# StefanSko/mcmc-db

Hardware: AMD Instinct MI355X
Metric: validated param-draws/sec (higher is better)
Workload: dtype f64; 1 GPU; single posteriordb-shaped model, 4x10000x100 synthetic draws per GPU (BASELINE config 1; AR(1) chains, ties and a shifted chain; SURVEY 8(d) C1); layout=pcn, statistics=mean,std,q5,q50,q95,split_rhat,ess_bulk,ess_tail

## Files before the change

include/mcmcref_hip.h:

```cpp
#ifndef MCMCREF_HIP_H
#define MCMCREF_HIP_H

#include <stddef.h>
#include <stdint.h>

#ifdef __cplusplus
extern "C" {
#endif

#define MCR_VERSION 100

#define MCR_OK 0
#define MCR_EINVAL (-1)
#define MCR_EMINCHAINS (-2)
#define MCR_EMINCHAINS_ARG (-3)
#define MCR_ENONFINITE (-4)
#define MCR_EHIP (-5)
#define MCR_ENOMEM (-6)
#define MCR_ENODEVICE (-7)
#define MCR_ECOMM (-8)
#define MCR_ELAYOUT (-9)
#define MCR_EFALLBACK (-10)

#define MCR_F64 0
// ... 8 lines not shown
    double* std;
    double* q;
    double* median;
    double* rhat;
    double* rhat_bulk;
    double* rhat_tail;
    double* ess_bulk;
    double* ess_tail;
    int64_t* lag_bulk;
    int64_t* lag_tail;
    int64_t* q_lo;
} mcr_summary;

typedef struct mcr_kernel_time {
    char name[48];
    int64_t launches;
    double total_ms;
} mcr_kernel_time;

int mcr_version(void);
int mcr_device_count(void);
int mcr_init(int device, mcr_ctx** out);
void mcr_free(mcr_ctx* ctx);
const char* mcr_last_error(const mcr_ctx* ctx);
int mcr_set_workspace_limit(mcr_ctx* ctx, size_t bytes);

int mcr_plan_chunks(mcr_ctx* ctx, int64_t C, int64_t N, int64_t P, int64_t stride_c, int64_t stride_n, int64_t stride_p,
                    int diagnostics, int64_t* params_per_chunk);

int mcr_plan_chunks_chains(mcr_ctx* ctx, const int64_t* chain_off, int C, int64_t P, int diagnostics,
                           int64_t* params_per_chunk);

int mcr_rho_guard_count(mcr_ctx* ctx, int64_t* rederived);

int mcr_dev_alloc(mcr_ctx* ctx, size_t bytes, void** dptr);
int mcr_dev_free(mcr_ctx* ctx, void* dptr);
int mcr_memcpy_h2d(mcr_ctx* ctx, void* dptr, const void* hptr, size_t bytes);
int mcr_memcpy_d2h(mcr_ctx* ctx, void* hptr, const void* dptr, size_t bytes);
int mcr_sync(mcr_ctx* ctx);

int mcr_summarize(mcr_ctx* ctx, const void* draws, int dtype, int64_t C, int64_t N, int64_t P,
                  int64_t stride_c, int64_t stride_n, int64_t stride_p, int min_chains,
                  const double* quantiles, int n_q, mcr_summary* out);
int mcr_summarize_dev(mcr_ctx* ctx, const void* draws_dev, int dtype, int64_t C, int64_t N,
                      int64_t P, int64_t stride_c, int64_t stride_n, int64_t stride_p,
                      int min_chains, const double* quantiles, int n_q, mcr_summary* out);
#define MCR_MAX_INFLIGHT 8
int mcr_summarize_enqueue(mcr_ctx* ctx, const void* draws_dev, int dtype, int64_t C, int64_t N,
                          int64_t P, int64_t stride_c, int64_t stride_n, int64_t stride_p,
                          int min_chains, const double* quantiles, int n_q, mcr_summary* out);
int mcr_summarize_wait(mcr_ctx* ctx);
int mcr_summarize_wait_one(mcr_ctx* ctx);

typedef struct mcr_model_desc {
    const void* draws_dev;
    int dtype;
    int min_chains;
    int64_t C, N, P;
    int64_t stride_c, stride_n, stride_p;
} mcr_model_desc;
int mcr_summarize_models(mcr_ctx* ctx, const mcr_model_desc* models, int n_models, const double* quantiles,
                         int n_q, mcr_summary* outs);

int mcr_diagnose_chains(mcr_ctx* ctx, const double* pooled, const int64_t* chain_off, int C,
                        int min_chains, mcr_summary* out, double* z_bulk, double* z_tail,
                        double* rank_bulk, double* rank_tail);
// ... 247 lines not shown
```

mcmc-db_amd/csrc/mcr_api.hip:

```cpp
#include "../../include/mcmcref_hip.h"

#include <hip/hip_runtime.h>

#include <algorithm>
#include <cmath>
#include <cstdarg>
#include <cstdio>
#include <cstdlib>
#include <cstring>
#include <fcntl.h>
#include <sys/stat.h>
#include <unistd.h>
#include <atomic>
#include <chrono>
#include <exception>
#include <memory>
#include <thread>
#include <unordered_map>
#include <string>
#include <functional>
#include <new>
#include <vector>

#include "mcr_kernels.hpp"
// ... 549 lines not shown
    if (lds_spl > 60 * 1024)
        HIP_TRY(ctx, hipFuncSetAttribute(reinterpret_cast<const void*>(&k_splitters<KT, MVT>),
                                         hipFuncAttributeMaxDynamicSharedMemorySize, (int)lds_spl));
    LAUNCH(ctx, K_SPLITTERS, (k_splitters<KT, MVT>), dim3((unsigned)a.pc), dim3(1024), lds_spl, keys, (const double*)a.samp,
           a.M, a.bk_k, a.bk_B, a.bk_D, a.bk_R, a.cut, a.boff);
    return MCR_OK;
}
template <typename KT>
int launch_splitters(mcr_ctx* ctx, const PipeIn& a, const KT* keys)
{
    const int S = a.bk_k * (int)(a.bk_R / 64);
    if (S <= 1024 || ctx->splitters_pairwise) return launch_splitters_v<KT, 0>(ctx, a, keys);
    if (S <= 2048) return launch_splitters_v<KT, 2>(ctx, a, keys);
    if (S <= 4096) return launch_splitters_v<KT, 4>(ctx, a, keys);
    return launch_splitters_v<KT, 8>(ctx, a, keys);
}

struct Sorted {
    double* keys; void* pos;
    double* keys_free; void* pos_free;
    bool ranked;
};

template <typename IdxT>
int sort_stage_t(mcr_ctx* ctx, PipeIn& a, Sorted& out)
{
    const i64 M = a.M, pc = a.pc;
    const unsigned py = (unsigned)pc;
    constexpr size_t lds_tile = sort_lds_bytes<IdxT>(kTile);
    const bool bucket = a.bk_B > 0;
    double* const samp1 = (bucket && a.bk_R == kTile) ? a.samp : (double*)nullptr;
    if (a.x_f32) {
        LAUNCH(ctx, K_TILE_SORT, (k_tile_sort<kTileNT, kTileVT, IdxT, float>), dim3((unsigned)a.ntiles, py), dim3(kTileNT),
               lds_tile, (const float*)a.X, M, a.kA, (IdxT*)a.iA, a.part, (int)a.ntiles, samp1);
    } else {
        LAUNCH(ctx, K_TILE_SORT, (k_tile_sort<kTileNT, kTileVT, IdxT, double>), dim3((unsigned)a.ntiles, py), dim3(kTileNT),
               lds_tile, (const double*)a.X, M, a.kA, (IdxT*)a.iA, a.part, (int)a.ntiles, samp1);
    }
    double *kin = a.kA, *kout = a.kB;
    IdxT *iin = (IdxT*)a.iA, *iout = (IdxT*)a.iB;
    const unsigned nblk = (unsigned)((M + kTile - 1) / kTile);
    const i64 Rstop = bucket ? a.bk_R : M;
    for (i64 R = kTile; R < Rstop; R *= 2) {
        LAUNCH(ctx, K_MERGE, (k_merge<kMergeNT, kMergeVT, false, IdxT>), dim3(nblk, py), dim3(kMergeNT), lds_tile + 256,
               (const double*)kin, (const IdxT*)iin, kout, iout, M, R, (double*)nullptr, pc,
               QArgs{}, (u32*)nullptr, (const i64*)nullptr);
        std::swap(kin, kout);
        std::swap(iin, iout);
    }
    if (bucket) {
        if (a.bk_R != kTile)
            LAUNCH(ctx, K_SPLITTERS, k_sample_runs<double>, dim3((unsigned)a.bk_k, py), dim3(256), 0, (const double*)kin, M,
                   a.bk_R, a.samp);
        {
            const int rc = launch_splitters<double>(ctx, a, (const double*)kin);
            if (rc) return rc;
        }
        const unsigned pgrp = (unsigned)((pc + 7) / 8 * 8);
        LAUNCH(ctx, K_BUCKET_MERGE, (k_bucket_merge<kMergeNT, kMergeVT, IdxT>), dim3(pgrp * (unsigned)a.bk_B), dim3(kMergeNT),
               lds_tile, (const double*)kin, (const IdxT*)iin, kout, iout, M, a.bk_k, a.bk_B, (const u32*)a.cut,
               (const u32*)a.boff, a.do_diag ? a.zb : (u32*)nullptr, pc, a.bk_R);
        std::swap(kin, kout);
        std::swap(iin, iout);
    }
    out = Sorted{kin, iin, kout, iout, bucket};
    return MCR_OK;
}

int sort_stage_rec(mcr_ctx* ctx, PipeIn& a, Sorted& out)
{
// ... 499 lines not shown
        const int v = atoi(env);
        ctx->n_lanes = v < 1 ? 1 : (v > MCR_MAX_INFLIGHT ? MCR_MAX_INFLIGHT : v);
    }
    if (const char* env = getenv("MCR_IO_PIECE_KB")) {
        const long v = atol(env);
        ctx->io_piece = (size_t)(v < 64 ? 64 : (v > (1 << 20) ? (1 << 20) : v)) << 10;
    }
    if (const char* env = getenv("MCR_IO_THREADS")) {
        const int v = atoi(env);
        ctx->io_threads = v < 1 ? 1 : (v > 64 ? 64 : v);
    }
    e = hipSetDevice(device);
    for (int l = 0; l < ctx->n_lanes && e == hipSuccess; ++l)
        e = hipStreamCreateWithFlags(&ctx->lanes[l].stream, hipStreamNonBlocking);
    for (int l = 0; l < ctx->n_lanes && e == hipSuccess; ++l) {
        e = hipStreamCreateWithFlags(&ctx->lanes[l].aux, hipStreamNonBlocking);
        if (e == hipSuccess) e = hipEventCreateWithFlags(&ctx->lanes[l].fork, hipEventDisableTiming);
        if (e == hipSuccess) e = hipEventCreateWithFlags(&ctx->lanes[l].join, hipEventDisableTiming);
    }
    if (e == hipSuccess) e = hipStreamCreateWithFlags(&ctx->copy_stream, hipStreamNonBlocking);
    if (e != hipSuccess) {
        mcr_free(ctx);
        return fail(nullptr, MCR_EHIP, "device %d init failed: %s", device, hipGetErrorString(e));
    }
    use_lane(ctx, 0);
    size_t mb = 8192;
    if (const char* env = getenv("MCR_WORKSPACE_MB")) { const long v = atol(env); if (v > 0) mb = (size_t)v; }
    ctx->ws_limit = mb << 20;
    if (const char* env = getenv("MCR_F32_RECORDS")) ctx->f32_records = atoi(env) != 0;
    if (const char* env = getenv("MCR_FFT")) ctx->fft_on = atoi(env) != 0;
    if (const char* env = getenv("MCR_SPLITTERS_PAIRWISE")) ctx->splitters_pairwise = atoi(env) != 0;
    if (const char* env = getenv("MCR_FORK")) ctx->fork_lone = atoi(env) != 0;
    if (const char* env = getenv("MCR_RHO_BAND")) { const double v = atof(env); if (v >= 0.0 && v < 1.0) ctx->rho_band = v; }
    if (ctx->guard_count.reserve(ctx, sizeof(unsigned)) != MCR_OK ||
        hipMemsetAsync(ctx->guard_count.p, 0, sizeof(unsigned), ctx->stream) != hipSuccess ||
        hipStreamSynchronize(ctx->stream) != hipSuccess) {
        mcr_free(ctx);
        return fail(nullptr, MCR_ENOMEM, "device %d: cannot allocate the guard counter", device);
    }
    *out = ctx;
    return MCR_OK;
}

void mcr_free(mcr_ctx* ctx)
{
    if (!ctx) return;
    hipSetDevice(ctx->device);
    sync_all(ctx);
    prof_resolve(ctx);
    for (hipEvent_t e : ctx->free_ev) hipEventDestroy(e);
    for (Slot& s : ctx->slots) if (s.done) hipEventDestroy(s.done);
    if (ctx->copy_stream) hipStreamDestroy(ctx->copy_stream);
    delete ctx;
}

int mcr_rho_guard_count(mcr_ctx* ctx, int64_t* rederived)
{
    if (!ctx || !rederived) return fail(ctx, MCR_EINVAL, "NULL argument");
    hipSetDevice(ctx->device);
    sync_all(ctx);
    unsigned v = 0;
    HIP_TRY(ctx, hipMemcpy(&v, ctx->guard_count.p, sizeof(unsigned), hipMemcpyDeviceToHost));
    *rederived = (int64_t)v;
    return MCR_OK;
}

int mcr_set_workspace_limit(mcr_ctx* ctx, size_t bytes)
{
    if (!ctx) return fail(nullptr, MCR_EINVAL, "ctx is NULL");
    if (bytes < (1u << 20)) return fail(ctx, MCR_EINVAL, "workspace limit must be at least 1 MiB");
    ctx->ws_limit = bytes;
    return MCR_OK;
}

int mcr_plan_chunks(mcr_ctx* ctx, int64_t C, int64_t N, int64_t P, int64_t sc, int64_t sn, int64_t sp, int diagnostics,
                    int64_t* params_per_chunk)
{
    if (!ctx || !params_per_chunk) return fail(ctx, MCR_EINVAL, "mcr_plan_chunks: NULL argument");
    if (C <= 0 || N <= 0 || P <= 0) { *params_per_chunk = 0; return MCR_OK; }
    ChunkPlan cp;
    const int rc = plan_chunks(ctx, shape_regular(C, N), P, needs_ingest(C, N, P, sc, sn, sp), diagnostics != 0, cp);
    if (rc) return rc;
    *params_per_chunk = cp.pcmax;
    return MCR_OK;
}

int mcr_dev_alloc(mcr_ctx* ctx, size_t bytes, void** dptr)
{
    if (!ctx || !dptr) return fail(ctx, MCR_EINVAL, "NULL argument");
    HIP_TRY(ctx, hipSetDevice(ctx->device));
    HIP_TRY(ctx, hipMalloc(dptr, bytes ? bytes : 1));
    return MCR_OK;
}
int mcr_dev_free(mcr_ctx* ctx, void* dptr)
{
    if (!ctx) return fail(nullptr, MCR_EINVAL, "ctx is NULL");
// ... 2980 lines not shown
```

mcmc-db_amd/csrc/mcr_kernels.hpp:

```cpp
#pragma once
#include <type_traits>
#include "mcr_device.hpp"
#include "mcr_sortnet.h"

namespace mcr {

enum ResField {
    R_MEAN = 0, R_STD, R_MEDIAN, R_RHAT, R_RHAT_BULK, R_RHAT_TAIL, R_ESS_BULK, R_ESS_TAIL,
    R_LAG_BULK, R_LAG_TAIL, R_BAD, R_Q0
};

#ifndef MCR_WCOMB
#define MCR_WCOMB 1
#endif
constexpr bool kWriteCombine = MCR_WCOMB != 0;

struct QArgs {
    int nq;
    i64 lo[32];
    double g[32];
    const void* xt = nullptr;
    int xf32 = 0;
};

// ... 264 lines not shown
    constexpr unsigned long long kLowQuads = 0x0F0F0F0F0F0F0F0Full;
    lane_pair_stage<0x141, true, kLowQuads>(k, ix);
    lane_pair_stage<0x4E, false, kLowPairs>(k, ix);
    lane_pair_stage<0xB1, false, kEvenLanes>(k, ix);
    lane_bitonic_merge16(k, ix);
#endif
}

template <int VT>
__device__ __forceinline__ void serial_merge(const double* skey, int a0, int na, int b0, int nb, int ai,
                                             int bi, int nout, double (&k)[VT], int (&src)[VT])
{
    int pa = a0 + ai, pb = b0 + bi;
    const int ea = a0 + na, eb = b0 + nb;
    double ak = skey[pos16(pa)], bk = skey[pos16(pb)];
#pragma unroll
    for (int i = 0; i < VT; ++i) {
        if (i < nout) {
            const bool takeA = (pb >= eb) | ((pa < ea) & !(bk < ak));
            k[i] = takeA ? ak : bk;
            src[i] = takeA ? pa : pb;
            pa += takeA ? 1 : 0;
            pb += takeA ? 0 : 1;
            const int pn = takeA ? pa : pb;
            const double nv = skey[pos16(pn)];
            ak = takeA ? nv : ak;
            bk = takeA ? bk : nv;
        } else {
            src[i] = 0;
        }
    }
}

template <typename IdxT> constexpr size_t sort_lds_bytes(int T) { return (size_t)T * (8 + sizeof(IdxT)); }

template <int NT, int VT, typename IdxT, typename XT>
__global__ __launch_bounds__(NT) void k_tile_sort(const XT* __restrict__ X, i64 M,
                                                  double* __restrict__ keys, IdxT* __restrict__ idx,
                                                  double* __restrict__ part, int ntiles,
                                                  double* __restrict__ samp)
{
    constexpr int T = NT * VT;
    extern __shared__ __attribute__((aligned(16))) char smem[];
    double* skey = reinterpret_cast<double*>(smem);
    IdxT* sidx = reinterpret_cast<IdxT*>(skey + T);
    double* red = skey;

    const int tid = threadIdx.x, tile = blockIdx.x;
    const i64 p = blockIdx.y;
    const i64 base = (i64)tile * T;
    const int count = (int)((M - base < (i64)T) ? M - base : (i64)T);
    const XT* src = X + p * M + base;

    const bool full = count == T;
    double k[VT];
    u32 ix[VT];
    double bad = 0.0;
    auto load = [&](auto full_c) {
        constexpr bool FULL = decltype(full_c)::value;
#pragma unroll
        for (int i = 0; i < VT; ++i) {
            const int e = i * NT + tid;
            const bool live = FULL || e < count;
            const double v = (double)src[FULL ? e : min(e, count - 1)];
            k[i] = live ? v : INFINITY;
            ix[i] = live ? (u32)(base + e) : 0xFFFFFFFFu;
            bad += (live && !isfinite(v)) ? 1.0 : 0.0;
        }
    };
    if (full) load(std::true_type{}); else load(std::false_type{});
    thread_sort<VT>(k, ix);
    constexpr bool kLaneLevels = MCR_TILE_DPP_LEVELS >= 2 && VT == 16;
    if constexpr (kLaneLevels) lane_merge_levels_16_to_64(k, ix);
// ... 25 lines not shown
            sidx[posi(e)] = (IdxT)ix[i];
        }
        __syncthreads();
    }

    auto write_out = [&](auto full_c) {
        constexpr bool FULL = decltype(full_c)::value;
#pragma nounroll
        for (int e = tid; e < (FULL ? T : count); e += NT) {
            keys[p * M + base + e] = skey[pos16(e)];
            idx[p * M + base + e] = sidx[posi(e)];
        }
    };
    if (full) write_out(std::true_type{}); else write_out(std::false_type{});
    if (samp != nullptr && tid < T / 64) {
        const int e = 64 * tid + 63;
        samp[(p * ntiles + tile) * (T / 64) + tid] = (e < count) ? skey[pos16(e)] : INFINITY;
    }
    __syncthreads();
    double s1 = 0.0, s2 = 0.0, e1 = 0.0, mt = 0.0;
    auto moments = [&](auto full_c) {
        constexpr bool FULL = decltype(full_c)::value;
        const int nlive = count - tid * VT;
#pragma unroll
        for (int i = 0; i < VT; ++i) s1 += (FULL || i < nlive) ? k[i] : 0.0;
        s1 = block_sum<NT>(s1, red);
        mt = s1 / (double)count;
#pragma unroll
        for (int i = 0; i < VT; ++i) { const double d = (FULL || i < nlive) ? k[i] - mt : 0.0; s2 = fma(d, d, s2); e1 += d; }
    };
    if (full) moments(std::true_type{}); else moments(std::false_type{});
    block_sum3<NT>(s2, e1, bad, red);
    if (tid == 0) store_slice_moments(part + (p * ntiles + tile) * kMomRec, mt, e1, s2, bad, (double)count);
}

template <int NT, int VT>
__device__ __forceinline__ void scatter_codes_by_line(u32* __restrict__ zrow, i64 M, int total, const u32 (&hcode)[VT],
                                                      const u32 (&hpos)[VT], u32* cnt_code, unsigned short* spos, u32* swt)
{
    constexpr int kMaxLines = 2048, PER = kMaxLines / NT > 0 ? kMaxLines / NT : 1;
    static_assert(NT * PER >= kMaxLines, "every line counter has an owner in the scan");
    const int tid = threadIdx.x;
    const int nlines = (int)((M + 31) >> 5);
    u32* scnt = cnt_code;
    u32* scode = cnt_code + 2112;
    __syncthreads();
    for (int i = tid; i <= nlines; i += NT) scnt[i] = 0u;
    __syncthreads();
    u32 rk[VT];
#pragma unroll
    for (int i = 0; i < VT; ++i) rk[i] = (tid * VT + i < total) ? atomicAdd(&scnt[hpos[i] >> 5], 1u) : 0u;
    __syncthreads();
    {
        u32 c[PER], tsum = 0;
#pragma unroll
        for (int j = 0; j < PER; ++j) { const int q = tid * PER + j; c[j] = (q < nlines) ? scnt[q] : 0u; tsum += c[j]; }
        u32 wtot;
        const u32 wex = wave_excl_scan_u32(tsum, wtot);
        if ((tid & 63) == 0) swt[tid >> 6] = wtot;
        __syncthreads();
        u32 base = wex;
        for (int w = 0; w < (tid >> 6); ++w) base += swt[w];
#pragma unroll
        for (int j = 0; j < PER; ++j) { const int q = tid * PER + j; if (q < nlines) scnt[q] = base; base += c[j]; }
    }
    __syncthreads();
// ... 777 lines not shown
```

mcmc-db_amd/csrc/mcr_sort32.hpp:

```cpp
#pragma once
#include "mcr_kernels.hpp"

namespace mcr {

__device__ __forceinline__ u32 rec_key(u64 r) { return (u32)(r >> 32); }
__device__ __forceinline__ u32 rec_pos(u64 r) { return (u32)r; }

template <int VT>
__device__ __forceinline__ void thread_sort_rec(u64 (&r)[VT])
{
    static_assert(VT == 16 || VT == 8, "sorting networks exist for 16 and 8 items per lane");
#define MCR_CE(a, b)                                         \
    {                                                        \
        const bool sw = r[b] < r[a];                         \
        const u64 lo = sw ? r[b] : r[a], hi = sw ? r[a] : r[b]; \
        r[a] = lo; r[b] = hi;                                \
    }
    if constexpr (VT == 16) { MCR_NET16(MCR_CE) } else { MCR_NET8(MCR_CE) }
#undef MCR_CE
}

template <int CTRL>
__device__ __forceinline__ u64 dpp_u64(u64 v)
{
    return ((u64)dpp_u32<CTRL>((u32)(v >> 32)) << 32) | (u64)dpp_u32<CTRL>((u32)v);
}
__device__ __forceinline__ u64 select_by_mask(u64 a, u64 b, unsigned long long m)
{
    return ((u64)select_by_mask((u32)(a >> 32), (u32)(b >> 32), m) << 32) | (u64)select_by_mask((u32)a, (u32)b, m);
}

template <int CTRL, bool MIRROR, unsigned long long MIN_LANES>
__device__ __forceinline__ void lane_pair_stage_rec(u64 (&r)[16])
{
    auto exchange = [](u64& own, u64 o) {
        const unsigned long long lt = __builtin_amdgcn_ballot_w64(o < own), gt = __builtin_amdgcn_ballot_w64(own < o);
        own = select_by_mask(own, o, (lt & MIN_LANES) | (gt & ~MIN_LANES));
    };
#pragma unroll
    for (int i = 0; i < (MIRROR ? 8 : 16); ++i) {
        const int s = MIRROR ? 15 - i : i;
        const u64 o_i = dpp_u64<CTRL>(r[s]);
        if (MIRROR) {
            const u64 o_s = dpp_u64<CTRL>(r[i]);
            exchange(r[s], o_s);
        }
        exchange(r[i], o_i);
    }
}

__device__ __forceinline__ void lane_bitonic_merge16_rec(u64 (&r)[16])
{
#define MCR_CE(a, b)                                         \
    {                                                        \
        const bool sw = r[b] < r[a];                         \
        const u64 lo = sw ? r[b] : r[a], hi = sw ? r[a] : r[b]; \
        r[a] = lo; r[b] = hi;                                \
    }
    MCR_BITONIC16(MCR_CE)
#undef MCR_CE
}

__device__ __forceinline__ void lane_merge_levels_rec(u64 (&r)[16])
{
    constexpr unsigned long long kEvenLanes = 0x5555555555555555ull, kLowPairs = 0x3333333333333333ull,
                                 kLowQuads = 0x0F0F0F0F0F0F0F0Full;
    lane_pair_stage_rec<0xB1, true, kEvenLanes>(r);
    lane_bitonic_merge16_rec(r);
    lane_pair_stage_rec<0x1B, true, kLowPairs>(r);
    lane_pair_stage_rec<0xB1, false, kEvenLanes>(r);
    lane_bitonic_merge16_rec(r);
    lane_pair_stage_rec<0x141, true, kLowQuads>(r);
    lane_pair_stage_rec<0x4E, false, kLowPairs>(r);
    lane_pair_stage_rec<0xB1, false, kEvenLanes>(r);
    lane_bitonic_merge16_rec(r);
}

template <int VT, int LIM = 0>
__device__ __forceinline__ void serial_merge_rec(const u64* srec, int a0, int na, int b0, int nb, int ai, int bi,
                                                 int nout, u64 (&out)[VT])
{
    int pa = a0 + ai, pb = b0 + bi;
    const int ea = a0 + na, eb = b0 + nb;
    auto slot = [](int e) { return pos16(LIM > 0 ? min(e, LIM) : e); };
    u64 ar = srec[slot(pa)], br = srec[slot(pb)];
#pragma unroll
    for (int i = 0; i < VT; ++i) {
        if (i < nout) {
            const bool takeA = (pb >= eb) | ((pa < ea) & !(br < ar));
            out[i] = takeA ? ar : br;
            pa += takeA ? 1 : 0;
            pb += takeA ? 0 : 1;
            const int pn = takeA ? pa : pb;
            const u64 nv = srec[slot(pn)];
            ar = takeA ? nv : ar;
            br = takeA ? br : nv;
        } else {
            out[i] = kRecPad;
        }
    }
}

constexpr size_t rec_lds_bytes(int T) { return (size_t)(T + 2) * 8; }

template <int NT, int VT>
__global__ __launch_bounds__(NT) void k_tile_sort32(const float* __restrict__ X, i64 M, u64* __restrict__ recs,
                                                    double* __restrict__ part, int ntiles, double* __restrict__ samp)
{
    constexpr int T = NT * VT;
    extern __shared__ __attribute__((aligned(16))) char smem[];
    u64* srec = reinterpret_cast<u64*>(smem);
    double* red = reinterpret_cast<double*>(smem);

    const int tid = threadIdx.x, tile = blockIdx.x;
    const i64 p = blockIdx.y;
    const i64 base = (i64)tile * T;
    const int count = (int)((M - base < (i64)T) ? M - base : (i64)T);
    const float* src = X + p * M + base;

    const bool full = count == T;
    u64 r[VT];
    double bad = 0.0;
    auto load = [&](auto full_c) {
        constexpr bool FULL = decltype(full_c)::value;
#pragma unroll
        for (int i = 0; i < VT; ++i) {
            const int e = i * NT + tid;
            const bool live = FULL || e < count;
            const float v = src[FULL ? e : min(e, count - 1)];
            bad += (live && !isfinite(v)) ? 1.0 : 0.0;
            r[i] = live ? (((u64)f32_key(v) << 32) | (u64)(u32)(base + e)) : kRecPad;
        }
    };
    if (full) load(std::true_type{}); else load(std::false_type{});
// ... 251 lines not shown
```

mcmc-db_amd/mcmc_ref_hip/_ffi.py:

```python
from __future__ import annotations

import collections
import contextlib
import ctypes as C
import math
import os
import threading
import time
from pathlib import Path

import numpy as np

MCR_OK = 0
MCR_EINVAL, MCR_EMINCHAINS, MCR_EMINCHAINS_ARG, MCR_ENONFINITE = -1, -2, -3, -4
MCR_EHIP, MCR_ENOMEM, MCR_ENODEVICE, MCR_ECOMM, MCR_ELAYOUT = -5, -6, -7, -8, -9
MCR_EFALLBACK = -10
MCR_F64, MCR_F32 = 0, 1
MCR_MAX_QUANTILES = 32
MCR_MAX_INFLIGHT = 8

_PKG = Path(__file__).resolve().parent
DEFAULT_LIB = _PKG.parent / "lib" / "libmcmcref_hip.so"


# ... 48 lines not shown


class PqColumn(C.Structure):
    _fields_ = [("name", C.c_char_p), ("type", C.c_int), ("src_kind", C.c_int), ("src_dev", C.c_void_p),
                ("stride", C.c_int64), ("seq_div", C.c_int64), ("seq_mod", C.c_int64)]


def pq_column(name: str, type_: int, src, stride: int = 1, kind: int | None = None) -> tuple:
    return (name, type_, kind, src, stride, 1, 1)


def pq_sequence(name: str, type_: int, div: int = 1, mod: int = INT64_MAX) -> tuple:
    return (name, type_, MCR_PQW_SEQ, None, 0, div, mod)


class IdColumns(C.Structure):
    _fields_ = [("chain_dev", C.c_void_p), ("draw_dev", C.c_void_p), ("rows", C.c_int64)]


class KernelTime(C.Structure):
    _fields_ = [("name", C.c_char * 48), ("launches", C.c_int64), ("total_ms", C.c_double)]


_I64 = C.c_int64
_TENSOR = [C.c_void_p, C.c_int, _I64, _I64, _I64, _I64, _I64, _I64]
SYMBOLS = {
    "mcr_version": (C.c_int, []),
    "mcr_device_count": (C.c_int, []),
    "mcr_init": (C.c_int, [C.c_int, C.POINTER(C.c_void_p)]),
    "mcr_free": (None, [C.c_void_p]),
    "mcr_last_error": (C.c_char_p, [C.c_void_p]),
    "mcr_set_workspace_limit": (C.c_int, [C.c_void_p, C.c_size_t]),
    "mcr_rho_guard_count": (C.c_int, [C.c_void_p, C.POINTER(C.c_int64)]),
    "mcr_plan_chunks": (C.c_int, [C.c_void_p] + [C.c_int64] * 6 + [C.c_int, C.POINTER(C.c_int64)]),
    "mcr_plan_chunks_chains": (C.c_int, [C.c_void_p, _ip, C.c_int, _I64, C.c_int, C.POINTER(C.c_int64)]),
    "mcr_dev_alloc": (C.c_int, [C.c_void_p, C.c_size_t, C.POINTER(C.c_void_p)]),
    "mcr_dev_free": (C.c_int, [C.c_void_p, C.c_void_p]),
    "mcr_memcpy_h2d": (C.c_int, [C.c_void_p, C.c_void_p, C.c_void_p, C.c_size_t]),
    "mcr_memcpy_d2h": (C.c_int, [C.c_void_p, C.c_void_p, C.c_void_p, C.c_size_t]),
    "mcr_sync": (C.c_int, [C.c_void_p]),
    "mcr_summarize": (C.c_int, [C.c_void_p] + _TENSOR + [C.c_int, _dp, C.c_int, C.POINTER(Summary)]),
    "mcr_summarize_dev": (C.c_int, [C.c_void_p] + _TENSOR + [C.c_int, _dp, C.c_int, C.POINTER(Summary)]),
    "mcr_summarize_enqueue": (C.c_int, [C.c_void_p] + _TENSOR + [C.c_int, _dp, C.c_int, C.POINTER(Summary)]),
    "mcr_summarize_models": (C.c_int, [C.c_void_p, C.POINTER(ModelDesc), C.c_int, _dp, C.c_int, C.POINTER(Summary)]),
    "mcr_summarize_wait": (C.c_int, [C.c_void_p]),
    "mcr_summarize_wait_one": (C.c_int, [C.c_void_p]),
    "mcr_diagnose_chains": (C.c_int, [C.c_void_p, _dp, _ip, C.c_int, C.c_int, C.POINTER(Summary),
                                      _dp, _dp, _dp, _dp]),
    "mcr_summarize_chains_enqueue": (C.c_int, [C.c_void_p, C.c_void_p, _I64, _ip, C.c_int, _I64, C.c_int, _dp, C.c_int,
                                               C.POINTER(Summary)]),
    "mcr_summarize_chains_dev": (C.c_int, [C.c_void_p, C.c_void_p, _I64, _ip, C.c_int, _I64, C.c_int, _dp, C.c_int,
                                           C.POINTER(Summary)]),
    "mcr_basic_stats": (C.c_int, [C.c_void_p, C.c_void_p, C.c_int, _I64, _dp, _dp]),
    "mcr_moments_dev": (C.c_int, [C.c_void_p] + _TENSOR + [_dp, _dp]),
    "mcr_compare": (C.c_int, [C.c_void_p, _dp, _dp, _I64, C.c_double, _dp, C.POINTER(C.c_uint8)]),
    "mcr_two_sample": (C.c_int, [C.c_void_p, _dp, _I64, _dp, _I64, _I64, _dp, _dp]),
    "mcr_sliced_two_sample": (C.c_int, [C.c_void_p, _dp, _I64, _dp, _I64, _I64, _dp, _dp, _I64, _dp, _dp, _dp, _dp]),
    "mcr_sliced_two_sample_dev": (C.c_int, [C.c_void_p, C.c_void_p, _I64, C.c_void_p, _I64, _I64, _dp, _dp, _I64, _dp, _dp,
                                            _dp, _dp]),
    "mcr_sliced_plan": (C.c_int, [C.c_void_p, _I64, _I64, _I64, _I64, C.POINTER(C.c_int64)]),
    "mcr_nested_rhat": (C.c_int, [C.c_void_p] + _TENSOR + [C.POINTER(C.c_int32), C.POINTER(Nested)]),
    "mcr_nested_rhat_dev": (C.c_int, [C.c_void_p] + _TENSOR + [C.POINTER(C.c_int32), C.POINTER(Nested)]),
    "mcr_nested_plan": (C.c_int, [C.c_void_p, C.c_int] + [_I64] * 7 + [C.POINTER(C.c_int64)]),
    "mcr_covariance": (C.c_int, [C.c_void_p, _dp, _I64, _I64, _dp]),
    "mcr_covariance_dev": (C.c_int, [C.c_void_p, C.c_void_p, _I64, _I64, C.c_void_p]),
    "mcr_profile_enable": (C.c_int, [C.c_void_p, C.c_int]),
# ... 929 lines not shown
        arrs = {n: np.full(max(P, 1), np.nan) for n in NESTED_FIELDS}
        out = Nested(**{n: _as_dp(a) for n, a in arrs.items()})
        self._check(fn(self.handle, ptr, *targs, ids.ctypes.data_as(C.POINTER(C.c_int32)), C.byref(out)))
        return {n: a[:P] for n, a in arrs.items()}

    def nested_params_per_chunk(self, t: "DeviceTensor", K: int) -> int:
        v = C.c_int64(0)
        self._check(self.lib.mcr_nested_plan(self.handle, *t.targs, int(K), C.byref(v)))
        return int(v.value)

    def covariance(self, draws) -> np.ndarray:
        x = np.ascontiguousarray(draws, dtype=np.float64)
        if x.ndim != 2:
            raise ValueError("draws must be 2-D [P][M]")
        P = x.shape[0]
        cov = np.full((max(P, 1), max(P, 1)), np.nan)
        self._check(self.lib.mcr_covariance(self.handle, _as_dp(x), x.shape[1], P, _as_dp(cov)))
        return cov[:P, :P] if P else np.empty((0, 0))

    def params_per_chunk(self, t: "DeviceTensor", diagnostics: bool = True) -> int:
        _, C_, N, P, sc, sn, sp = t.targs
        v = C.c_int64(0)
        if t.chain_off is not None:
            self._check(self.lib.mcr_plan_chunks_chains(self.handle, _as_ip(t.chain_off), C_, P, int(diagnostics), C.byref(v)))
            return int(v.value)
        self._check(self.lib.mcr_plan_chunks(self.handle, C_, N, P, sc, sn, sp, int(diagnostics), C.byref(v)))
        return int(v.value)

    def rho_guard_count(self) -> int:
        v = C.c_int64(0)
        self._check(self.lib.mcr_rho_guard_count(self.handle, C.byref(v)))
        return int(v.value)

    def profile(self, on: bool):
        self._check(self.lib.mcr_profile_enable(self.handle, 1 if on else 0))

    def profile_reset(self):
        self._check(self.lib.mcr_profile_reset(self.handle))

    def profile_get(self) -> dict:
        arr = (KernelTime * 64)()
        n = C.c_int(0)
        self._check(self.lib.mcr_profile_get(self.handle, arr, 64, C.byref(n)))
        return {arr[i].name.decode(): {"launches": int(arr[i].launches), "total_ms": float(arr[i].total_ms)}
                for i in range(min(n.value, 64))}


def pipeline(ctx: Context, jobs, owns: bool = False):
    if ctx.inflight:
        ctx.wait()
    window = collections.deque()
    try:
        for tag, t, kw in jobs:
            try:
                window.append((tag, t, ctx.enqueue(t, **kw)))
            except McrError as exc:
                window.append((tag, t, exc))
            if len(window) == MCR_MAX_INFLIGHT:
                yield _retire(ctx, window, owns)
        while window:
            yield _retire(ctx, window, owns)
    finally:
        if window:
            try:
                ctx.wait()
            except McrError:
# ... 66 lines not shown
```

Before: 26.37 billion param-draws/s.

## Sort tile keys as packed 64-bit records with slot index, fallback on violations

The tile sort now packs each key and its 12-bit tile slot into a single double-sized record. The sorting network, DPP lane merges and LDS merge passes therefore move one 8-byte value instead of a key plus a separate index. The dropped low mantissa bits are restored afterwards from a side LDS array. If the rebuilt keys are not in order, the tile is re-sorted with the original key/index path and a device counter is incremented. Compare-exchange uses v_min/v_max f64, and the kernel is given a waves-per-EU hint; the cost is extra validation and possible double work on tiles with ties in the high bits.

```diff
diff --git a/include/mcmcref_hip.h b/include/mcmcref_hip.h
--- a/include/mcmcref_hip.h
+++ b/include/mcmcref_hip.h
@@ -64,6 +64,8 @@
                            int64_t* params_per_chunk);
 
 int mcr_rho_guard_count(mcr_ctx* ctx, int64_t* rederived);
+
+int mcr_tile_fallback_count(mcr_ctx* ctx, int64_t* tiles);
 
 int mcr_dev_alloc(mcr_ctx* ctx, size_t bytes, void** dptr);
 int mcr_dev_free(mcr_ctx* ctx, void* dptr);
diff --git a/mcmc-db_amd/csrc/mcr_api.hip b/mcmc-db_amd/csrc/mcr_api.hip
--- a/mcmc-db_amd/csrc/mcr_api.hip
+++ b/mcmc-db_amd/csrc/mcr_api.hip
@@ -605,10 +605,12 @@
     double* const samp1 = (bucket && a.bk_R == kTile) ? a.samp : (double*)nullptr;
     if (a.x_f32) {
         LAUNCH(ctx, K_TILE_SORT, (k_tile_sort<kTileNT, kTileVT, IdxT, float>), dim3((unsigned)a.ntiles, py), dim3(kTileNT),
-               lds_tile, (const float*)a.X, M, a.kA, (IdxT*)a.iA, a.part, (int)a.ntiles, samp1);
+               lds_tile, (const float*)a.X, M, a.kA, (IdxT*)a.iA, a.part, (int)a.ntiles, samp1,
+               ctx->guard_count.as<unsigned>() + 1);
     } else {
         LAUNCH(ctx, K_TILE_SORT, (k_tile_sort<kTileNT, kTileVT, IdxT, double>), dim3((unsigned)a.ntiles, py), dim3(kTileNT),
-               lds_tile, (const double*)a.X, M, a.kA, (IdxT*)a.iA, a.part, (int)a.ntiles, samp1);
+               lds_tile, (const double*)a.X, M, a.kA, (IdxT*)a.iA, a.part, (int)a.ntiles, samp1,
+               ctx->guard_count.as<unsigned>() + 1);
     }
     double *kin = a.kA, *kout = a.kB;
     IdxT *iin = (IdxT*)a.iA, *iout = (IdxT*)a.iB;
@@ -1174,8 +1176,8 @@
     if (const char* env = getenv("MCR_SPLITTERS_PAIRWISE")) ctx->splitters_pairwise = atoi(env) != 0;
     if (const char* env = getenv("MCR_FORK")) ctx->fork_lone = atoi(env) != 0;
     if (const char* env = getenv("MCR_RHO_BAND")) { const double v = atof(env); if (v >= 0.0 && v < 1.0) ctx->rho_band = v; }
-    if (ctx->guard_count.reserve(ctx, sizeof(unsigned)) != MCR_OK ||
-        hipMemsetAsync(ctx->guard_count.p, 0, sizeof(unsigned), ctx->stream) != hipSuccess ||
+    if (ctx->guard_count.reserve(ctx, 2 * sizeof(unsigned)) != MCR_OK ||
+        hipMemsetAsync(ctx->guard_count.p, 0, 2 * sizeof(unsigned), ctx->stream) != hipSuccess ||
         hipStreamSynchronize(ctx->stream) != hipSuccess) {
         mcr_free(ctx);
         return fail(nullptr, MCR_ENOMEM, "device %d: cannot allocate the guard counter", device);
@@ -1204,6 +1206,17 @@
     unsigned v = 0;
     HIP_TRY(ctx, hipMemcpy(&v, ctx->guard_count.p, sizeof(unsigned), hipMemcpyDeviceToHost));
     *rederived = (int64_t)v;
+    return MCR_OK;
+}
+
+int mcr_tile_fallback_count(mcr_ctx* ctx, int64_t* tiles)
+{
+    if (!ctx || !tiles) return fail(ctx, MCR_EINVAL, "NULL argument");
+    hipSetDevice(ctx->device);
+    sync_all(ctx);
+    unsigned v = 0;
+    HIP_TRY(ctx, hipMemcpy(&v, ctx->guard_count.as<unsigned>() + 1, sizeof(unsigned), hipMemcpyDeviceToHost));
+    *tiles = (int64_t)v;
     return MCR_OK;
 }
 
diff --git a/mcmc-db_amd/csrc/mcr_kernels.hpp b/mcmc-db_amd/csrc/mcr_kernels.hpp
--- a/mcmc-db_amd/csrc/mcr_kernels.hpp
+++ b/mcmc-db_amd/csrc/mcr_kernels.hpp
@@ -320,13 +320,22 @@
     }
 }
 
+#ifndef MCR_TILE_REC
+#define MCR_TILE_REC 1
+#endif
+#if MCR_TILE_REC == 0
+#define MCR_TILE_PAIRS_INLINE __forceinline__
+#else
+#define MCR_TILE_PAIRS_INLINE __noinline__
+#endif
+
 template <typename IdxT> constexpr size_t sort_lds_bytes(int T) { return (size_t)T * (8 + sizeof(IdxT)); }
 
 template <int NT, int VT, typename IdxT, typename XT>
-__global__ __launch_bounds__(NT) void k_tile_sort(const XT* __restrict__ X, i64 M,
-                                                  double* __restrict__ keys, IdxT* __restrict__ idx,
-                                                  double* __restrict__ part, int ntiles,
-                                                  double* __restrict__ samp)
+__device__ MCR_TILE_PAIRS_INLINE void tile_sort_pairs(const XT* __restrict__ X, i64 M,
+                                                      double* __restrict__ keys, IdxT* __restrict__ idx,
+                                                      double* __restrict__ part, int ntiles,
+                                                      double* __restrict__ samp)
 {
     constexpr int T = NT * VT;
     extern __shared__ __attribute__((aligned(16))) char smem[];
@@ -418,6 +427,271 @@
     if (full) moments(std::true_type{}); else moments(std::false_type{});
     block_sum3<NT>(s2, e1, bad, red);
     if (tid == 0) store_slice_moments(part + (p * ntiles + tile) * kMomRec, mt, e1, s2, bad, (double)count);
+}
+
+#ifndef MCR_TILE_REC_MINMAX
+#define MCR_TILE_REC_MINMAX 1
+#endif
+template <typename R> __device__ __forceinline__ R rec_pad();
+template <> __device__ __forceinline__ u64 rec_pad<u64>() { return kRecPad; }
+template <> __device__ __forceinline__ double rec_pad<double>() { return INFINITY; }
+
+__device__ __forceinline__ void rec_ce(u64& a, u64& b)
+{
+    const bool sw = b < a;
+    const u64 lo = sw ? b : a, hi = sw ? a : b;
+    a = lo; b = hi;
+}
+__device__ __forceinline__ void rec_ce(double& a, double& b)
+{
+#if MCR_TILE_REC_MINMAX
+    double lo, hi;
+    asm("v_min_f64 %0, %1, %2" : "=v"(lo) : "v"(a), "v"(b));
+    asm("v_max_f64 %0, %1, %2" : "=v"(hi) : "v"(a), "v"(b));
+    a = lo; b = hi;
+#else
+    const bool sw = b < a;
+    const double lo = sw ? b : a, hi = sw ? a : b;
+    a = lo; b = hi;
+#endif
+}
+
+template <int VT, typename R>
+__device__ __forceinline__ void thread_sort_rec(R (&r)[VT])
+{
+    static_assert(VT == 16 || VT == 8, "sorting networks exist for 16 and 8 items per lane");
+#define MCR_CE(a, b) rec_ce(r[a], r[b]);
+    if constexpr (VT == 16) { MCR_NET16(MCR_CE) } else { MCR_NET8(MCR_CE) }
+#undef MCR_CE
+}
+
+template <int CTRL>
+__device__ __forceinline__ u64 dpp_rec(u64 v)
+{
+    return ((u64)dpp_u32<CTRL>((u32)(v >> 32)) << 32) | (u64)dpp_u32<CTRL>((u32)v);
+}
+template <int CTRL>
+__device__ __forceinline__ double dpp_rec(double v) { return dpp_f64<CTRL>(v); }
+__device__ __forceinline__ u64 select_by_mask(u64 a, u64 b, unsigned long long m)
+{
+    return ((u64)select_by_mask((u32)(a >> 32), (u32)(b >> 32), m) << 32) | (u64)select_by_mask((u32)a, (u32)b, m);
+}
+
+template <int CTRL, bool MIRROR, unsigned long long MIN_LANES, typename R>
+__device__ __forceinline__ void lane_pair_stage_rec(R (&r)[16])
+{
+    auto exchange = [](R& own, R o) {
+        const unsigned long long lt = __builtin_amdgcn_ballot_w64(o < own), gt = __builtin_amdgcn_ballot_w64(own < o);
+        own = select_by_mask(own, o, (lt & MIN_LANES) | (gt & ~MIN_LANES));
+    };
+#pragma unroll
+    for (int i = 0; i < (MIRROR ? 8 : 16); ++i) {
+        const int s = MIRROR ? 15 - i : i;
+        const R o_i = dpp_rec<CTRL>(r[s]);
+        if (MIRROR) {
+            const R o_s = dpp_rec<CTRL>(r[i]);
+            exchange(r[s], o_s);
+        }
+        exchange(r[i], o_i);
+    }
+}
+
+template <typename R>
+__device__ __forceinline__ void lane_bitonic_merge16_rec(R (&r)[16])
+{
+#define MCR_CE(a, b) rec_ce(r[a], r[b]);
+    MCR_BITONIC16(MCR_CE)
+#undef MCR_CE
+}
+
+template <typename R>
+__device__ __forceinline__ void lane_merge_levels_rec(R (&r)[16])
+{
+    constexpr unsigned long long kEvenLanes = 0x5555555555555555ull, kLowPairs = 0x3333333333333333ull,
+                                 kLowQuads = 0x0F0F0F0F0F0F0F0Full;
+    lane_pair_stage_rec<0xB1, true, kEvenLanes>(r);
+    lane_bitonic_merge16_rec(r);
+    lane_pair_stage_rec<0x1B, true, kLowPairs>(r);
+    lane_pair_stage_rec<0xB1, false, kEvenLanes>(r);
+    lane_bitonic_merge16_rec(r);
+    lane_pair_stage_rec<0x141, true, kLowQuads>(r);
+    lane_pair_stage_rec<0x4E, false, kLowPairs>(r);
+    lane_pair_stage_rec<0xB1, false, kEvenLanes>(r);
+    lane_bitonic_merge16_rec(r);
+}
+
+template <int VT, int LIM = 0, typename R>
+__device__ __forceinline__ void serial_merge_rec(const R* srec, int a0, int na, int b0, int nb, int ai, int bi,
+                                                 int nout, R (&out)[VT])
+{
+    int pa = a0 + ai, pb = b0 + bi;
+    const int ea = a0 + na, eb = b0 + nb;
+    auto slot = [](int e) { return pos16(LIM > 0 ? min(e, LIM) : e); };
+    R ar = srec[slot(pa)], br = srec[slot(pb)];
+#pragma unroll
+    for (int i = 0; i < VT; ++i) {
+        if (i < nout) {
+            const bool takeA = (pb >= eb) | ((pa < ea) & !(br < ar));
+            out[i] = takeA ? ar : br;
+            pa += takeA ? 1 : 0;
+            pb += takeA ? 0 : 1;
+            const int pn = takeA ? pa : pb;
+            const R nv = srec[slot(pn)];
+            ar = takeA ? nv : ar;
+            br = takeA ? br : nv;
+        } else {
+            out[i] = rec_pad<R>();
+        }
+    }
+}
+
+template <int NT, int VT, typename IdxT, typename XT>
+__global__ __launch_bounds__(NT) __attribute__((amdgpu_waves_per_eu(4))) void k_tile_sort(const XT* __restrict__ X, i64 M,
+                                                  double* __restrict__ keys, IdxT* __restrict__ idx,
+                                                  double* __restrict__ part, int ntiles,
+                                                  double* __restrict__ samp, unsigned* __restrict__ fallbacks)
+{
+#if MCR_TILE_REC == 0
+    tile_sort_pairs<NT, VT, IdxT, XT>(X, M, keys, idx, part, ntiles, samp);
+#else
+    constexpr int T = NT * VT;
+    constexpr u32 kSlotMask = 0xFFFu;
+    static_assert(T <= 4096, "a record has 12 bits for the tile slot");
+    extern __shared__ __attribute__((aligned(16))) char smem[];
+    double* srec = reinterpret_cast<double*>(smem);
+    unsigned short* slow = reinterpret_cast<unsigned short*>(srec + T);
+    IdxT* sidx = reinterpret_cast<IdxT*>(srec + T);
+    double* red = srec;
+
+    const int tid = threadIdx.x, tile = blockIdx.x;
+    const i64 p = blockIdx.y;
+    const i64 base = (i64)tile * T;
+    const int count = (int)((M - base < (i64)T) ? M - base : (i64)T);
+    const XT* src = X + p * M + base;
+    const bool full = count == T;
+    const int nlive = count - tid * VT;
+
+    double r[VT];
+    double bad = 0.0;
+    auto load = [&](auto full_c) {
+        constexpr bool FULL = decltype(full_c)::value;
+        XT v[VT];
+#pragma unroll
+        for (int i = 0; i < VT; ++i) {
+            const int e = i * NT + tid;
+            v[i] = src[FULL ? e : min(e, count - 1)];
+        }
+#pragma unroll
+        for (int i = 0; i < VT; ++i) {
+            const int e = i * NT + tid;
+            const bool live = FULL || e < count;
+            const double d = (double)v[i];
+            const bool fin = isfinite(d);
+            bad += (live && !fin) ? 1.0 : 0.0;
+            const u32 lo = (u32)__double2loint(d), hi = (u32)__double2hiint(d);
+            if (live) slow[e] = (unsigned short)(lo & kSlotMask);
+            const double rec = __hiloint2double((int)(fin ? hi : 0u), (int)((lo & ~kSlotMask) | (u32)e));
+            r[i] = live ? rec : INFINITY;
+        }
+    };
+    if (full) load(std::true_type{}); else load(std::false_type{});
+    thread_sort_rec<VT>(r);
+    static_assert(MCR_TILE_DPP_LEVELS == 0 || MCR_TILE_DPP_LEVELS >= 3,
+                  "the record sort has all three register levels or none: build MCR_TILE_DPP_LEVELS=2 with MCR_TILE_REC=0");
+    constexpr bool kLaneLevels = MCR_TILE_DPP_LEVELS >= 3 && VT == 16;
+    if constexpr (kLaneLevels) lane_merge_levels_rec(r);
+#pragma unroll
+    for (int i = 0; i < VT; ++i) srec[pos16(tid * VT + i)] = r[i];
+    __syncthreads();
+    for (int coop = kLaneLevels ? 16 : 2; coop <= NT; coop <<= 1) {
+        const int first = tid & ~(coop - 1);
+        const int run = VT * (coop >> 1);
+        const int a0 = first * VT, b0 = a0 + run;
+        const int diag = VT * (tid - first);
+        auto A = [&](int i) { return srec[pos16(a0 + i)]; };
+        auto B = [&](int j) { return srec[pos16(b0 + j)]; };
+        const int ai = merge_path32(A, run, B, run, diag);
+        serial_merge_rec<VT>(srec, a0, run, b0, run, ai, diag - ai, VT, r);
+        __syncthreads();
+        if (coop < NT) {
+#pragma unroll
+            for (int i = 0; i < VT; ++i) srec[pos16(tid * VT + i)] = r[i];
+            __syncthreads();
+        }
+    }
+
+    double k[VT];
+    u32 slot[VT];
+    bool viol = false;
+    auto rebuild = [&](auto full_c) {
+        constexpr bool FULL = decltype(full_c)::value;
+#pragma unroll
+        for (int i = 0; i < VT; ++i) {
+            const u32 lo = (u32)__double2loint(r[i]);
+            slot[i] = lo & kSlotMask;
+            const double key = __hiloint2double(__double2hiint(r[i]), (int)((lo & ~kSlotMask) | (u32)slow[slot[i]]));
+            k[i] = (FULL || i < nlive) ? key : INFINITY;
+        }
+    };
+    if (full) rebuild(std::true_type{}); else rebuild(std::false_type{});
+#pragma unroll
+    for (int i = 0; i + 1 < VT; ++i) viol |= k[i + 1] < k[i];
+    constexpr int NW = NT / kWave;
+    const int lane = tid & (kWave - 1), wave = tid / kWave;
+    const double next_first = dpp_f64<0x130>(k[0]);
+    viol |= lane + 1 < kWave && next_first < k[VT - 1];
+    int* wflag = reinterpret_cast<int*>(srec + 2 * NW);
+    const bool wave_viol = __builtin_amdgcn_ballot_w64(viol) != 0;
+    if (lane == 0) { srec[wave] = k[0]; wflag[wave] = wave_viol ? 1 : 0; }
+    if (lane == kWave - 1) srec[NW + wave] = k[VT - 1];
+    __syncthreads();
+    bool fall = MCR_TILE_REC == 2;
+#pragma unroll
+    for (int w = 0; w < NW; ++w) {
+        fall |= wflag[w] != 0;
+        if (w + 1 < NW) fall |= srec[w + 1] < srec[NW + w];
+    }
+    __syncthreads();
+    if (fall) {
+        if (tid == 0 && fallbacks != nullptr) atomicAdd(fallbacks, 1u);
+        tile_sort_pairs<NT, VT, IdxT, XT>(X, M, keys, idx, part, ntiles, samp);
+        return;
+    }
+#pragma unroll
+    for (int i = 0; i < VT; ++i) {
+        srec[pos16(tid * VT + i)] = k[i];
+        sidx[posi(tid * VT + i)] = (IdxT)((u32)base + slot[i]);
+    }
+    __syncthreads();
+
+    auto write_out = [&](auto full_c) {
+        constexpr bool FULL = decltype(full_c)::value;
+#pragma nounroll
+        for (int e = tid; e < (FULL ? T : count); e += NT) {
+            keys[p * M + base + e] = srec[pos16(e)];
+            idx[p * M + base + e] = sidx[posi(e)];
+        }
+    };
+    if (full) write_out(std::true_type{}); else write_out(std::false_type{});
+    if (samp != nullptr && tid < T / 64) {
+        const int e = 64 * tid + 63;
+        samp[(p * ntiles + tile) * (T / 64) + tid] = (e < count) ? srec[pos16(e)] : INFINITY;
+    }
+    __syncthreads();
+    double s1 = 0.0, s2 = 0.0, e1 = 0.0, mt = 0.0;
+    auto moments = [&](auto full_c) {
+        constexpr bool FULL = decltype(full_c)::value;
+#pragma unroll
+        for (int i = 0; i < VT; ++i) s1 += (FULL || i < nlive) ? k[i] : 0.0;
+        s1 = block_sum<NT>(s1, red);
+        mt = s1 / (double)count;
+#pragma unroll
+        for (int i = 0; i < VT; ++i) { const double d = (FULL || i < nlive) ? k[i] - mt : 0.0; s2 = fma(d, d, s2); e1 += d; }
+    };
+    if (full) moments(std::true_type{}); else moments(std::false_type{});
+    block_sum3<NT>(s2, e1, bad, red);
+    if (tid == 0) store_slice_moments(part + (p * ntiles + tile) * kMomRec, mt, e1, s2, bad, (double)count);
+#endif
 }
 
 template <int NT, int VT>
diff --git a/mcmc-db_amd/csrc/mcr_sort32.hpp b/mcmc-db_amd/csrc/mcr_sort32.hpp
--- a/mcmc-db_amd/csrc/mcr_sort32.hpp
+++ b/mcmc-db_amd/csrc/mcr_sort32.hpp
@@ -6,100 +6,6 @@
 __device__ __forceinline__ u32 rec_key(u64 r) { return (u32)(r >> 32); }
 __device__ __forceinline__ u32 rec_pos(u64 r) { return (u32)r; }
 
-template <int VT>
-__device__ __forceinline__ void thread_sort_rec(u64 (&r)[VT])
-{
-    static_assert(VT == 16 || VT == 8, "sorting networks exist for 16 and 8 items per lane");
-#define MCR_CE(a, b)                                         \
-    {                                                        \
-        const bool sw = r[b] < r[a];                         \
-        const u64 lo = sw ? r[b] : r[a], hi = sw ? r[a] : r[b]; \
-        r[a] = lo; r[b] = hi;                                \
-    }
-    if constexpr (VT == 16) { MCR_NET16(MCR_CE) } else { MCR_NET8(MCR_CE) }
-#undef MCR_CE
-}
-
-template <int CTRL>
-__device__ __forceinline__ u64 dpp_u64(u64 v)
-{
-    return ((u64)dpp_u32<CTRL>((u32)(v >> 32)) << 32) | (u64)dpp_u32<CTRL>((u32)v);
-}
-__device__ __forceinline__ u64 select_by_mask(u64 a, u64 b, unsigned long long m)
-{
-    return ((u64)select_by_mask((u32)(a >> 32), (u32)(b >> 32), m) << 32) | (u64)select_by_mask((u32)a, (u32)b, m);
-}
-
-template <int CTRL, bool MIRROR, unsigned long long MIN_LANES>
-__device__ __forceinline__ void lane_pair_stage_rec(u64 (&r)[16])
-{
-    auto exchange = [](u64& own, u64 o) {
-        const unsigned long long lt = __builtin_amdgcn_ballot_w64(o < own), gt = __builtin_amdgcn_ballot_w64(own < o);
-        own = select_by_mask(own, o, (lt & MIN_LANES) | (gt & ~MIN_LANES));
-    };
-#pragma unroll
-    for (int i = 0; i < (MIRROR ? 8 : 16); ++i) {
-        const int s = MIRROR ? 15 - i : i;
-        const u64 o_i = dpp_u64<CTRL>(r[s]);
-        if (MIRROR) {
-            const u64 o_s = dpp_u64<CTRL>(r[i]);
-            exchange(r[s], o_s);
-        }
-        exchange(r[i], o_i);
-    }
-}
-
-__device__ __forceinline__ void lane_bitonic_merge16_rec(u64 (&r)[16])
-{
-#define MCR_CE(a, b)                                         \
-    {                                                        \
-        const bool sw = r[b] < r[a];                         \
-        const u64 lo = sw ? r[b] : r[a], hi = sw ? r[a] : r[b]; \
-        r[a] = lo; r[b] = hi;                                \
-    }
-    MCR_BITONIC16(MCR_CE)
-#undef MCR_CE
-}
-
-__device__ __forceinline__ void lane_merge_levels_rec(u64 (&r)[16])
-{
-    constexpr unsigned long long kEvenLanes = 0x5555555555555555ull, kLowPairs = 0x3333333333333333ull,
-                                 kLowQuads = 0x0F0F0F0F0F0F0F0Full;
-    lane_pair_stage_rec<0xB1, true, kEvenLanes>(r);
-    lane_bitonic_merge16_rec(r);
-    lane_pair_stage_rec<0x1B, true, kLowPairs>(r);
-    lane_pair_stage_rec<0xB1, false, kEvenLanes>(r);
-    lane_bitonic_merge16_rec(r);
-    lane_pair_stage_rec<0x141, true, kLowQuads>(r);
-    lane_pair_stage_rec<0x4E, false, kLowPairs>(r);
-    lane_pair_stage_rec<0xB1, false, kEvenLanes>(r);
-    lane_bitonic_merge16_rec(r);
-}
-
-template <int VT, int LIM = 0>
-__device__ __forceinline__ void serial_merge_rec(const u64* srec, int a0, int na, int b0, int nb, int ai, int bi,
-                                                 int nout, u64 (&out)[VT])
-{
-    int pa = a0 + ai, pb = b0 + bi;
-    const int ea = a0 + na, eb = b0 + nb;
-    auto slot = [](int e) { return pos16(LIM > 0 ? min(e, LIM) : e); };
-    u64 ar = srec[slot(pa)], br = srec[slot(pb)];
-#pragma unroll
-    for (int i = 0; i < VT; ++i) {
-        if (i < nout) {
-            const bool takeA = (pb >= eb) | ((pa < ea) & !(br < ar));
-            out[i] = takeA ? ar : br;
-            pa += takeA ? 1 : 0;
-            pb += takeA ? 0 : 1;
-            const int pn = takeA ? pa : pb;
-            const u64 nv = srec[slot(pn)];
-            ar = takeA ? nv : ar;
-            br = takeA ? br : nv;
-        } else {
-            out[i] = kRecPad;
-        }
-    }
-}
 
 constexpr size_t rec_lds_bytes(int T) { return (size_t)(T + 2) * 8; }
 
diff --git a/mcmc-db_amd/mcmc_ref_hip/_ffi.py b/mcmc-db_amd/mcmc_ref_hip/_ffi.py
--- a/mcmc-db_amd/mcmc_ref_hip/_ffi.py
+++ b/mcmc-db_amd/mcmc_ref_hip/_ffi.py
@@ -104,6 +104,7 @@
     "mcr_last_error": (C.c_char_p, [C.c_void_p]),
     "mcr_set_workspace_limit": (C.c_int, [C.c_void_p, C.c_size_t]),
     "mcr_rho_guard_count": (C.c_int, [C.c_void_p, C.POINTER(C.c_int64)]),
+    "mcr_tile_fallback_count": (C.c_int, [C.c_void_p, C.POINTER(C.c_int64)]),
     "mcr_plan_chunks": (C.c_int, [C.c_void_p] + [C.c_int64] * 6 + [C.c_int, C.POINTER(C.c_int64)]),
     "mcr_plan_chunks_chains": (C.c_int, [C.c_void_p, _ip, C.c_int, _I64, C.c_int, C.POINTER(C.c_int64)]),
     "mcr_dev_alloc": (C.c_int, [C.c_void_p, C.c_size_t, C.POINTER(C.c_void_p)]),
@@ -1099,6 +1100,11 @@
         self._check(self.lib.mcr_rho_guard_count(self.handle, C.byref(v)))
         return int(v.value)
 
+    def tile_fallback_count(self) -> int:
+        v = C.c_int64(0)
+        self._check(self.lib.mcr_tile_fallback_count(self.handle, C.byref(v)))
+        return int(v.value)
+
     def profile(self, on: bool):
         self._check(self.lib.mcr_profile_enable(self.handle, 1 if on else 0))
 
```

Measured after the change: 26.83 billion param-draws/s, median of 6. 1.7% higher.
